# c0rv4x/zkevm-prover

Measured on AMD Instinct MI355X. Metric: batch-proof STARK sec (2^23 trace) + Goldilocks NTT Gelem/s at 1/2/4/8 GPU, lower is better.
Workload: dtype u64 (Goldilocks) + F_p^3

## Files before the change

### include/zkgpu.h

```cpp
#ifndef ZKGPU_H
#define ZKGPU_H

#include <stdint.h>
#include "zkgpu_zxp.h"

#ifdef __cplusplus
extern "C" {
#endif

#define ZKGPU_OK 0
#define ZKGPU_ERR_HIP -1
#define ZKGPU_ERR_ARG -2
#define ZKGPU_ERR_INIT -3
#define ZKGPU_ERR_OOM -4

int zkgpu_init(int device);
void zkgpu_release(void);
const char *zkgpu_last_error(void);
int zkgpu_set_stream(void *hip_stream);
void *zkgpu_get_stream(void);
int zkgpu_synchronize(void);
int zkgpu_abi_version(void);

int zkgpu_gl_ntt(uint64_t *dst, const uint64_t *src, uint64_t n, uint64_t ncols, int inverse);
// ... 126 lines not shown
                         const uint64_t *evals, uint32_t n_evals, char *buf, uint64_t buflen, int rtc_check);

int zkgpu_calculate_z_dev(uint64_t *z, uint64_t z_ld, const uint64_t *num, uint64_t num_ld, const uint64_t *den,
                          uint64_t den_ld, uint64_t n, int *closes);
int zkgpu_calculate_z_block_dev(uint64_t *z, uint64_t z_ld, const uint64_t *num, uint64_t num_ld, const uint64_t *den,
                                uint64_t den_ld, uint64_t n, const uint64_t z0[3], uint64_t total[3]);
typedef struct zkgpu_z_req {
    uint64_t *z;
    uint64_t z_ld;
    const uint64_t *num;
    uint64_t num_ld;
    const uint64_t *den;
    uint64_t den_ld;
} zkgpu_z_req;
int zkgpu_calculate_z_many_dev(const zkgpu_z_req *req, uint32_t nz, uint64_t n, int *closes);

int zkgpu_evmap_dev(uint64_t *evals_out, const uint64_t *const *cols, const uint64_t *lds, const uint32_t *dims,
                    const uint32_t *primes, uint32_t n_ev, const uint64_t *lev, const uint64_t *lpev, uint64_t l_ld,
                    uint64_t n, uint32_t extend_bits);

int zkgpu_xdivxsub_dev(uint64_t *xdiv, uint64_t *xdivw, const uint64_t xi[3], uint32_t n_bits, uint32_t n_bits_ext);
int zkgpu_xdivxsub_rows_dev(uint64_t *xdiv, uint64_t *xdivw, const uint64_t xi[3], uint32_t n_bits,
                            uint32_t n_bits_ext, uint64_t row0, uint64_t nrows);
int zkgpu_lagrange_xi_rows_dev(uint64_t *lev, uint64_t *lpev, uint64_t ld, const uint64_t xi[3], uint32_t n_bits,
                               uint64_t row0, uint64_t nrows);

int zkgpu_ext_powers_dev(uint64_t *out, uint64_t ld, const uint64_t base[3], uint64_t n);

int zkgpu_scale_by_powers_dev(uint64_t *cols, uint64_t ld, uint32_t ncols, uint64_t n, uint64_t base);

// ... 64 lines not shown
```

### zkevm-prover_amd/csrc/api.hip

```cpp
#include <stdarg.h>
#include <stdio.h>
#include <string.h>

#include <algorithm>
#include <deque>
#include <map>
#include <mutex>
#include <new>
#include <thread>
#include <vector>

#include "gl_device.hpp"
#include "zkgpu_internal.hpp"
#include "poseidon_gl_constants.h"
#include "poseidon_gl_sparse.h"

namespace zk {

int upload_poseidon_constants(Ctx &c);
int merkle_leaves_absorb(uint64_t *nodes, const uint64_t *src, uint64_t ld, uint64_t col0, uint64_t ncols,
                         uint64_t total, uint64_t nrows, hipStream_t s);

static Ctx g_ctx;
static thread_local char g_err[512] = "";
// ... 1164 lines not shown
int zkgpu_calculate_z_block_dev(uint64_t *z, uint64_t z_ld, const uint64_t *num, uint64_t num_ld, const uint64_t *den,
                                uint64_t den_ld, uint64_t n, const uint64_t z0[3], uint64_t total[3])
{
    int rc;
    if ((rc = require_init())) return rc;
    if (!z0 || !total) return set_error(ZKGPU_ERR_ARG, "calculate_z_block: null z0 / total");
    if (!n) {
        for (int k = 0; k < 3; k++) total[k] = z0[k] % HP;
        return 0;
    }
    if (z_ld < n || num_ld < n || den_ld < n) return set_error(ZKGPU_ERR_ARG, "calculate_z: ld < n");
    const size_t words = calculate_z_scratch_words(n);
    uint64_t *scr = workspace(2, (words + 8) * sizeof(uint64_t));
    if (!scr) return ZKGPU_ERR_OOM;
    uint64_t *tot = scr + words;
    if ((rc = calculate_z(z, z_ld, num, num_ld, den, den_ld, n, z0, scr, tot, g_ctx.stream))) return rc;
    if ((rc = check_hip(hipMemcpyAsync(total, tot, 24, hipMemcpyDeviceToHost, g_ctx.stream), "D2H"))) return rc;
    return check_hip(hipStreamSynchronize(g_ctx.stream), "calculateZ sync");
}

int zkgpu_calculate_z_many_dev(const zkgpu_z_req *req, uint32_t nz, uint64_t n, int *closes)
{
    int rc;
    if ((rc = require_init())) return rc;
    if (!nz) return 0;
    if (!req || !closes) return set_error(ZKGPU_ERR_ARG, "calculate_z_many: null argument");
    if (!n) {
        for (uint32_t k = 0; k < nz; k++) closes[k] = 1;
        return 0;
    }
    for (uint32_t k = 0; k < nz; k++)
        if (req[k].z_ld < n || req[k].num_ld < n || req[k].den_ld < n)
            return set_error(ZKGPU_ERR_ARG, "calculate_z_many: request %u: ld < n", k);
    const size_t words = calculate_z_scratch_words(n);
    uint64_t *scr = workspace(2, (words + 3ULL * nz + 8) * sizeof(uint64_t));
    if (!scr) return ZKGPU_ERR_OOM;
    uint64_t *tot = scr + words;
    const uint64_t one[3] = {1, 0, 0};
    for (uint32_t k = 0; k < nz; k++)
        if ((rc = calculate_z(req[k].z, req[k].z_ld, req[k].num, req[k].num_ld, req[k].den, req[k].den_ld, n, one, scr,
                              tot + 3ULL * k, g_ctx.stream)))
            return rc;
    std::vector<uint64_t> t(3ULL * nz);
    if ((rc = check_hip(hipMemcpyAsync(t.data(), tot, t.size() * 8, hipMemcpyDeviceToHost, g_ctx.stream), "D2H")))
        return rc;
    if ((rc = check_hip(hipStreamSynchronize(g_ctx.stream), "calculateZ sync"))) return rc;
    for (uint32_t k = 0; k < nz; k++) closes[k] = (t[3 * k] == 1 && t[3 * k + 1] == 0 && t[3 * k + 2] == 0) ? 1 : 0;
    return 0;
}

int zkgpu_calculate_z_dev(uint64_t *z, uint64_t z_ld, const uint64_t *num, uint64_t num_ld, const uint64_t *den,
                          uint64_t den_ld, uint64_t n, int *closes)
{
    const uint64_t one[3] = {1, 0, 0};
    uint64_t tot[3] = {1, 0, 0};
    const int rc = zkgpu_calculate_z_block_dev(z, z_ld, num, num_ld, den, den_ld, n, one, tot);
    if (rc) return rc;
// ... 490 lines not shown
```

### zkevm-prover_amd/csrc/stark.hip

```cpp
#include "gl_device.hpp"
#include "zkgpu_internal.hpp"
#include "../../include/zkgpu_zxp.h"

namespace zk {

template <int K>
__device__ __forceinline__ uint64_t sqr_n(uint64_t x)
{
#pragma unroll
    for (int i = 0; i < K; i++) x = gl_sqr(x);
    return x;
}

__device__ __forceinline__ uint64_t gl_inv_base(uint64_t x)
{
    uint64_t t2 = gl_mul(gl_sqr(x), x);
    uint64_t t3 = gl_mul(gl_sqr(t2), x);
    uint64_t t6 = gl_mul(sqr_n<3>(t3), t3);
    uint64_t t12 = gl_mul(sqr_n<6>(t6), t6);
    uint64_t t24 = gl_mul(sqr_n<12>(t12), t12);
    uint64_t t30 = gl_mul(sqr_n<6>(t24), t6);
    uint64_t t31 = gl_mul(gl_sqr(t30), x);
    uint64_t t32 = gl_mul(gl_sqr(t31), x);
    return gl_mul(sqr_n<33>(t31), t32);
}

__device__ __forceinline__ gl3 gl3_inv(const gl3 &a)
{
    uint64_t a0 = a.v[0], a1 = a.v[1], a2 = a.v[2];
    uint64_t s02 = gl_add(a0, a2), s12 = gl_add(a1, a2);
    uint64_t c0 = gl_sub(gl_mul(s02, s02), gl_mul(s12, a1));
    uint64_t c1 = gl_sub(gl_mul(s12, a2), gl_mul(a1, s02));
    uint64_t c2 = gl_sub(gl_mul(a1, a1), gl_mul(s02, a2));
    uint64_t det = gl_add(gl_add(gl_mul(a0, c0), gl_mul(a2, c1)), gl_mul(a1, c2));
    uint64_t di = gl_inv_base(det);
    return gl3{{gl_mul(c0, di), gl_mul(c1, di), gl_mul(c2, di)}};
}

__device__ __forceinline__ gl3 ld3(const uint64_t *p0, uint64_t ld)
{
    return gl3{{p0[0], p0[ld], p0[2 * ld]}};
}

__device__ __forceinline__ void st3(uint64_t *p0, uint64_t ld, const gl3 &v)
{
    p0[0] = gl_canon(v.v[0]);
    p0[ld] = gl_canon(v.v[1]);
    p0[2 * ld] = gl_canon(v.v[2]);
}

__device__ __forceinline__ uint64_t rand_u64(uint64_t seed, uint64_t stream, uint64_t col, uint64_t row)
// ... 282 lines not shown
__global__ void __launch_bounds__(ZXP_THREADS) k_zxp_eval_rows(ZxpEnv e, const uint64_t *rows, uint32_t n_rows)
{
    extern __shared__ __attribute__((aligned(16))) uint64_t zlds[];
    const int lane = threadIdx.x;
    const uint64_t j = (uint64_t)blockIdx.x * ZXP_THREADS + lane;
    const uint64_t i = j < n_rows ? rows[j] : ~0ULL;
    const bool active = i < (1ULL << e.logdom);
    if (!__ballot(active)) return;
    zxp_eval_body<true>(e, zlds, lane, i, active, j);
}

constexpr int BI_CHUNK = 16;
constexpr int SCAN_THREADS = 256;
constexpr int Z_PER = 4;
constexpr uint64_t Z_TILE = SCAN_THREADS * Z_PER;
__device__ __forceinline__ int z_slot(int e) { return e + e / Z_PER; }
constexpr int Z_SLOTS = Z_TILE + Z_TILE / Z_PER;

__device__ gl3 block_exclusive_scan3(gl3 v, gl3 *sh, gl3 *total)
{
    const int t = threadIdx.x;
    sh[t] = v;
    __syncthreads();
    for (int off = 1; off < SCAN_THREADS; off <<= 1) {
        gl3 x = sh[t];
        gl3 y = t >= off ? sh[t - off] : gl3{{1, 0, 0}};
        __syncthreads();
        sh[t] = t >= off ? gl3_mul(x, y) : x;
        __syncthreads();
    }
    gl3 excl = t ? sh[t - 1] : gl3{{1, 0, 0}};
    *total = sh[SCAN_THREADS - 1];
    __syncthreads();
    return excl;
}

__device__ __forceinline__ void lds_st3(uint64_t *img, int slot, const gl3 &v)
{
    img[slot] = v.v[0];
    img[Z_SLOTS + slot] = v.v[1];
    img[2 * Z_SLOTS + slot] = v.v[2];
}
__device__ __forceinline__ gl3 lds_ld3(const uint64_t *img, int slot)
{
    return gl3{{img[slot], img[Z_SLOTS + slot], img[2 * Z_SLOTS + slot]}};
}

__global__ void __launch_bounds__(SCAN_THREADS) k_z_ratio(uint64_t *ratio, uint64_t *thr_pre, uint64_t *tile_tot,
                                                          const uint64_t *num, uint64_t num_ld, const uint64_t *den,
                                                          uint64_t den_ld, uint64_t n)
{
    __shared__ uint64_t img[3 * Z_SLOTS];
    __shared__ gl3 sh[SCAN_THREADS];
    const int t = threadIdx.x;
    const uint64_t base = (uint64_t)blockIdx.x * Z_TILE;
    gl3 pre[Z_PER];
    gl3 acc{{1, 0, 0}};
#pragma unroll
    for (int j = 0; j < Z_PER; j++) {
        const uint64_t k = base + j * SCAN_THREADS + t;
        const gl3 d = k < n ? ld3(den + k, den_ld) : gl3{{1, 0, 0}};
        acc = j ? gl3_mul(acc, d) : d;
        pre[j] = acc;
    }
    gl3 inv = gl3_inv(acc);
#pragma unroll
    for (int jj = 0; jj < Z_PER; jj++) {
        const int j = Z_PER - 1 - jj;
        const int e = j * SCAN_THREADS + t;
        const uint64_t k = base + e;
        const gl3 dinv = j ? gl3_mul(inv, pre[j - 1]) : inv;
        gl3 r{{1, 0, 0}};
        if (k < n) {
            r = gl3_mul(ld3(num + k, num_ld), dinv);
            uint64_t *o = ratio + 3 * k;
            o[0] = r.v[0];
            o[1] = r.v[1];
            o[2] = r.v[2];
            if (j) inv = gl3_mul(inv, ld3(den + k, den_ld));
        }
        lds_st3(img, z_slot(e), r);
    }
    __syncthreads();
    gl3 run = lds_ld3(img, z_slot(t * Z_PER));
#pragma unroll
    for (int i = 1; i < Z_PER; i++) run = gl3_mul(run, lds_ld3(img, z_slot(t * Z_PER + i)));
    gl3 tot;
    const gl3 ex = block_exclusive_scan3(run, sh, &tot);
    uint64_t *tp = thr_pre + 3 * ((uint64_t)blockIdx.x * SCAN_THREADS + t);
    tp[0] = ex.v[0];
    tp[1] = ex.v[1];
    tp[2] = ex.v[2];
    if (t == 0) {
        tile_tot[3 * blockIdx.x] = tot.v[0];
        tile_tot[3 * blockIdx.x + 1] = tot.v[1];
        tile_tot[3 * blockIdx.x + 2] = tot.v[2];
    }
}

__global__ void __launch_bounds__(SCAN_THREADS) k_z_totals(uint64_t *tile_pre, const uint64_t *tile_tot,
                                                           uint64_t ntiles, gl3 z0, uint64_t *total)
{
    __shared__ gl3 sh[SCAN_THREADS];
    const uint64_t per = (ntiles + SCAN_THREADS - 1) / SCAN_THREADS;
    const uint64_t b0 = threadIdx.x * per;
    uint64_t b1 = b0 + per;
    if (b1 > ntiles) b1 = ntiles;
    gl3 acc{{1, 0, 0}};
    for (uint64_t b = b0; b < b1; b++) acc = gl3_mul(acc, ld3(tile_tot + 3 * b, 1));
    gl3 tot;
    gl3 run = gl3_mul(z0, block_exclusive_scan3(acc, sh, &tot));
    for (uint64_t b = b0; b < b1; b++) {
        tile_pre[3 * b] = run.v[0];
        tile_pre[3 * b + 1] = run.v[1];
        tile_pre[3 * b + 2] = run.v[2];
        run = gl3_mul(run, ld3(tile_tot + 3 * b, 1));
    }
    if (threadIdx.x == 0) {
        const gl3 t = gl3_canon(gl3_mul(z0, tot));
        total[0] = t.v[0];
        total[1] = t.v[1];
        total[2] = t.v[2];
    }
}

__global__ void __launch_bounds__(SCAN_THREADS) k_z_apply(uint64_t *z, uint64_t z_ld, const uint64_t *ratio,
                                                          const uint64_t *thr_pre, const uint64_t *tile_pre,
                                                          uint64_t n)
{
    __shared__ uint64_t img[3 * Z_SLOTS];
    const int t = threadIdx.x;
    const uint64_t base = (uint64_t)blockIdx.x * Z_TILE;
#pragma unroll
    for (int j = 0; j < Z_PER; j++) {
        const int e = j * SCAN_THREADS + t;
        const uint64_t k = base + e;
        lds_st3(img, z_slot(e), k < n ? ld3(ratio + 3 * k, 1) : gl3{{1, 0, 0}});
    }
    gl3 run = gl3_mul(ld3(tile_pre + 3 * blockIdx.x, 1), ld3(thr_pre + 3 * ((uint64_t)blockIdx.x * SCAN_THREADS + t), 1));
    __syncthreads();
#pragma unroll
    for (int i = 0; i < Z_PER; i++) {
        const int sl = z_slot(t * Z_PER + i);
        const gl3 r = lds_ld3(img, sl);
        lds_st3(img, sl, run);
        run = gl3_mul(run, r);
    }
    __syncthreads();
#pragma unroll
    for (int j = 0; j < Z_PER; j++) {
        const int e = j * SCAN_THREADS + t;
        const uint64_t k = base + e;
        if (k < n) st3(z + k, z_ld, lds_ld3(img, z_slot(e)));
    }
}

constexpr int EV_THREADS = 256;

constexpr int EV_G = 8;
constexpr uint64_t EV_ROWS_PER_THREAD = 240;
struct EvGroup {
    const uint64_t *col[EV_G];
    uint32_t prime, sub0;
};

template <int G, int U>
__global__ void __launch_bounds__(EV_THREADS) k_evmap_groups(uint64_t *partial, const EvGroup *groups,
                                                            const uint64_t *lev, const uint64_t *lpev, uint64_t l_ld,
// ... 66 lines not shown
    }
    acc = gl3_canon(acc);
    evals[3 * e] = acc.v[0];
    evals[3 * e + 1] = acc.v[1];
    evals[3 * e + 2] = acc.v[2];
}

template <bool INTERLEAVED>
__global__ void __launch_bounds__(256) k_xdiv_rows(uint64_t *out0, uint64_t *out1, uint64_t ld, gl3 a0, gl3 a1,
                                                   uint64_t shift, gl3 scale, uint32_t logn, uint64_t row0,
                                                   uint64_t nrows, const uint64_t *tw_lo, const uint64_t *tw_hi)
{
    const uint64_t n = 1ULL << logn;
    const uint64_t T = (uint64_t)gridDim.x * blockDim.x;
    const uint64_t t = (uint64_t)blockIdx.x * blockDim.x + threadIdx.x;
    for (int which = 0; which < 2; which++) {
        const gl3 s = which ? a1 : a0;
        uint64_t *out = which ? out1 : out0;
        gl3 pre[BI_CHUNK];
        uint64_t xs[BI_CHUNK];
        gl3 acc{{1, 0, 0}};
#pragma unroll
        for (int j = 0; j < BI_CHUNK; j++) {
            uint64_t k = t + j * T;
            uint64_t ex = ((row0 + k) & (n - 1)) << (TW_MAX_LOG - logn);
            xs[j] = gl_mul(shift, gl_mul(tw_lo[ex & (TW_LEVEL_SIZE - 1)], tw_hi[ex >> TW_LEVEL_BITS]));
            gl3 d = k < nrows ? gl3{{gl_sub(xs[j], s.v[0]), gl_neg(s.v[1]), gl_neg(s.v[2])}} : gl3{{1, 0, 0}};
            acc = j ? gl3_mul(acc, d) : d;
            pre[j] = acc;
        }
        gl3 inv = gl3_inv(acc);
#pragma unroll
        for (int jj = 0; jj < BI_CHUNK; jj++) {
            const int j = BI_CHUNK - 1 - jj;
            uint64_t k = t + j * T;
            gl3 dinv = j ? gl3_mul(inv, pre[j - 1]) : inv;
            if (k < nrows) {
                gl3 d{{gl_sub(xs[j], s.v[0]), gl_neg(s.v[1]), gl_neg(s.v[2])}};
                gl3 r = gl3_mul1(dinv, xs[j]);
                if constexpr (!INTERLEAVED) r = gl3_mul(r, scale);
                r = gl3_canon(r);
                if constexpr (INTERLEAVED) {
                    out[3 * k] = r.v[0];
                    out[3 * k + 1] = r.v[1];
                    out[3 * k + 2] = r.v[2];
                } else {
                    out[k] = r.v[0];
                    out[ld + k] = r.v[1];
                    out[2 * ld + k] = r.v[2];
                }
                inv = gl3_mul(inv, d);
            }
        }
    }
}

__device__ __forceinline__ gl3 gl3_pow(gl3 b, uint64_t e)
{
    gl3 r{{1, 0, 0}};
    while (e) {
        if (e & 1) r = gl3_mul(r, b);
        b = gl3_mul(b, b);
        e >>= 1;
    }
    return r;
}
// ... 132 lines not shown
    if (!n_rows) return 0;
    size_t lds;
    const ZxpEnv e = zxp_env(L, true, lds);
    prof_begin(s);
    hipLaunchKernelGGL(k_zxp_eval_rows, dim3(nblk(n_rows, ZXP_THREADS)), dim3(ZXP_THREADS), lds, s, e, rows, n_rows);
    prof_end("k_zxp_eval_rows", L.bytes, s);
    return check_launch("k_zxp_eval_rows");
}

size_t calculate_z_scratch_words(uint64_t n)
{
    const uint64_t nt = (n + Z_TILE - 1) / Z_TILE;
    return 3 * n + 3 * nt * SCAN_THREADS + 6 * nt + 4;
}

int calculate_z(uint64_t *z, uint64_t z_ld, const uint64_t *num, uint64_t num_ld, const uint64_t *den,
                uint64_t den_ld, uint64_t n, const uint64_t z0[3], uint64_t *scratch, uint64_t *total_dev, hipStream_t s)
{
    const uint64_t nt = (n + Z_TILE - 1) / Z_TILE;
    uint64_t *ratio = scratch;
    uint64_t *thr = ratio + 3 * n;
    uint64_t *tot = thr + 3 * nt * SCAN_THREADS;
    uint64_t *pre = tot + 3 * nt;
    prof_begin(s);
    hipLaunchKernelGGL(k_z_ratio, dim3((uint32_t)nt), dim3(SCAN_THREADS), 0, s, ratio, thr, tot, num, num_ld, den,
                       den_ld, n);
    prof_end("k_z_ratio", 8.0 * 9 * n, s);
    const gl3 z0v{{z0[0], z0[1], z0[2]}};
    hipLaunchKernelGGL(k_z_totals, dim3(1), dim3(SCAN_THREADS), 0, s, pre, tot, nt, z0v, total_dev);
    prof_begin(s);
    hipLaunchKernelGGL(k_z_apply, dim3((uint32_t)nt), dim3(SCAN_THREADS), 0, s, z, z_ld, ratio, thr, pre, n);
    prof_end("k_z_apply", 8.0 * 6 * n, s);
    return check_launch("calculateZ");
}

size_t evmap_group_size() { return sizeof(EvGroup); }
uint32_t evmap_group_width() { return EV_G; }
uint64_t evmap_rows_per_block() { return EV_ROWS_PER_THREAD * EV_THREADS; }

int evmap_groups(uint64_t *evals, const void *groups_dev, uint32_t n_groups, uint32_t width, uint32_t unroll,
                 const int32_t *subs_dev,
                 uint32_t n_ev, uint32_t n_sub, const uint64_t *lev, const uint64_t *lpev, uint64_t l_ld, uint64_t n,
                 uint32_t eb, uint64_t *partial, hipStream_t s)
{
    if (!n_ev) return 0;
    const uint64_t rpb = evmap_rows_per_block();
    const uint32_t nblk_ = (uint32_t)((n + rpb - 1) / rpb);
// ... 117 lines not shown
```

### zkevm-prover_amd/csrc/zkgpu_internal.hpp

```cpp
#pragma once
#include <hip/hip_runtime.h>
#include <stdint.h>

#include "../../include/zkgpu.h"
#include "../../include/zkgpu_zxp.h"
#include "zxp_jit_source.hpp"
#include "zxp_prepare.hpp"

namespace zk {

constexpr uint32_t NTT_MAX_PASSES = 4;
constexpr uint32_t POST_BITS = 12;

struct Workspace {
    void *ptr = nullptr;
    size_t bytes = 0;
};

struct Ctx {
    int device = -1;
    bool ready = false;
    hipStream_t stream = nullptr;
    uint64_t *rt_small[2] = {nullptr, nullptr};
    uint64_t *tw_lo[2] = {nullptr, nullptr};
// ... 50 lines not shown
int fri_fold_rows(uint64_t *out, const uint64_t *rows, uint64_t g0, uint64_t n_local, uint32_t pol_bits,
                  uint32_t out_bits, const uint64_t sx[3], uint64_t shift_inv, hipStream_t s);
int fri_transpose(uint64_t *aux, const uint64_t *pol, uint64_t degree, uint32_t tbits, hipStream_t s);

int zxp_jit_run(const ZxpJitIn &in, hipStream_t s);

int rand_cols(uint64_t *base, uint64_t ld, const uint32_t *cols_dev, uint32_t ncols, uint64_t nrows, uint64_t seed,
              uint64_t stream, uint64_t row0, uint64_t rmask, hipStream_t s);
int copy_rows(uint64_t *dst, uint64_t dld, uint64_t drow0, const uint32_t *dcols, const uint64_t *src, uint64_t sld,
              uint64_t srow0, uint64_t smask, const uint32_t *scols, uint32_t ncols, uint64_t nrows, hipStream_t s);
int zxp_eval(const ZxpLaunch &L, hipStream_t s);
int zxp_eval_rows(const ZxpLaunch &L, const uint64_t *rows, uint32_t n_rows, hipStream_t s);
uint32_t nonzero_rows_blocks(uint64_t n);
int nonzero_rows(uint64_t *out, uint32_t *counts, const uint64_t *cols, uint64_t ld, uint32_t ncols, uint64_t n,
                 uint32_t max_rows, hipStream_t s);
size_t calculate_z_scratch_words(uint64_t n);
int calculate_z(uint64_t *z, uint64_t z_ld, const uint64_t *num, uint64_t num_ld, const uint64_t *den,
                uint64_t den_ld, uint64_t n, const uint64_t z0[3], uint64_t *scratch, uint64_t *total_dev, hipStream_t s);
size_t evmap_group_size();
uint32_t evmap_group_width();
uint64_t evmap_rows_per_block();
int evmap_groups(uint64_t *evals, const void *groups_dev, uint32_t n_groups, uint32_t width, uint32_t unroll,
                 const int32_t *subs_dev,
                 uint32_t n_ev, uint32_t n_sub, const uint64_t *lev, const uint64_t *lpev, uint64_t l_ld, uint64_t n, uint32_t eb,
                 uint64_t *partial, hipStream_t s);
int xdivxsub(uint64_t *xdiv, uint64_t *xdivw, const uint64_t xi[3], uint64_t w, uint32_t logn, hipStream_t s);
int xdivxsub_rows(uint64_t *xdiv, uint64_t *xdivw, const uint64_t xi[3], uint64_t w, uint32_t logn, uint64_t row0,
                  uint64_t nrows, hipStream_t s);
int xdiv_rows(uint64_t *out0, uint64_t *out1, uint64_t ld, int interleaved, const uint64_t a0[3],
              const uint64_t a1[3], uint64_t shift, const uint64_t scale[3], uint32_t logn, uint64_t row0,
              uint64_t nrows, hipStream_t s);
int ext_powers(uint64_t *out, uint64_t ld, const uint64_t base[3], uint64_t n, hipStream_t s);
int scale_powers(uint64_t *cols, uint64_t ld, uint32_t ncols, uint64_t n, uint64_t base, hipStream_t s);
// ... 14 lines not shown
```

### zkevm-prover_amd/host/sharded_starks.hpp

```cpp

class ShardedStarks : public Starks
{
public:
    zkgpu_comm comm{};
    uint32_t W = 1, R = 0;
    uint64_t B = 0, H = 0, BH = 0;
    uint64_t hn = 0, ldn = 0;
    uint64_t *ext = nullptr;
    uint64_t *coln = nullptr;
    uint64_t *gath = nullptr;
    uint64_t *cm4 = nullptr;
    uint64_t *xchg = nullptr;
    uint64_t *hsend = nullptr, *hrecv = nullptr;
    uint64_t *pack_s = nullptr, *pack_r = nullptr;
    uint64_t *psend(uint32_t d) const { return pack_s + (uint64_t)(d < R ? d : d - 1) * stride_s; }
    uint64_t stride_s = 0, stride_r = 0;
    uint32_t max_ops = 0;
    uint64_t n_exch = 0, sent_bytes = 0, max_sent = 0;
    uint64_t *puw = nullptr;
    uint64_t *hs_send = nullptr, *hs_recv = nullptr, *hs_ret = nullptr, *hs_ret_in = nullptr, *hs_seg = nullptr;
    uint32_t *hs_cnt = nullptr, *hs_start = nullptr;
    uint64_t hs_recv_cap = 0;
    uint64_t slot = 0, hcap = 0;
    struct Tree {
// ... 181 lines not shown
        return 8 * ((coln_words() >= const_words() ? 0 : const_words()) + (ext_words() >= const_words() ? 0 : const_words()));
    }
    int setup_buffer(uint64_t **p, uint64_t *have, uint64_t cap, uint64_t words, void **owned)
    {
        *owned = nullptr;
        if (have && cap >= words) {
            *p = have;
            return 0;
        }
        CK(zkgpu_dev_malloc(owned, words * 8));
        *p = (uint64_t *)*owned;
        return 0;
    }
    uint64_t lde_cols_max() const override { return max_share(); }
    uint64_t prog_rows_max() const override { return std::max(B, nb); }

    uint64_t s0_record() const
    {
        return (uint64_t)info.n_cm1 + info.n_cm2 + info.n_cm3 + info.n_cm4 + info.n_const + 20ULL * info.n_bits_ext;
    }

    int exchange()
    {
        if (W == 1) {
            ops.clear();
            return 0;
        }
        max_ops = std::max(max_ops, (uint32_t)ops.size());
        if (ops.size() > 2ULL * (W - 1)) {
            const size_t n = ops.size();
// ... 850 lines not shown
```

### zkevm-prover_amd/host/starks.cpp

```cpp
#include <math.h>
#include <stdarg.h>
#include <stdio.h>
#include <stdlib.h>
#include <string.h>

#include <algorithm>
#include <chrono>
#include <map>
#include <string>
#include <vector>

#include "../../include/zkgpu.h"
#include "../../include/zkgpu_stark.h"
#include "zkgpu_audit_format.hpp"

namespace zkgpu_host {

static thread_local char g_err[512] = "";
static int fail(const char *fmt, ...)
{
    va_list ap;
    va_start(ap, fmt);
    vsnprintf(g_err, sizeof g_err, fmt, ap);
    va_end(ap);
// ... 179 lines not shown
        }
        void *v = nullptr;
        CK(zkgpu_dev_malloc(&v, elems * 8));
        allocs.push_back(v);
        CK(zkgpu_memset_dev(v, 0, elems * 8));
        *p = (uint64_t *)v;
        return 0;
    }

    virtual uint64_t setup_bytes() const { return 0; }
    virtual uint64_t lde_cols_max() const
    {
        return std::max({info.n_cm1, info.n_cm2, info.n_cm3, info.n_const, 1u});
    }
    virtual uint64_t prog_rows_max() const { return NE; }
    virtual uint64_t stream_stage_words() const
    {
        const uint64_t b = std::min<uint64_t>(std::max(info.n_cm1, 1u), 128);
        return 2 * std::min<uint64_t>(N * b, (64ULL << 20) / 8);
    }
    uint64_t lde_batch_cap = 0;
    int plan(uint64_t *bytes)
    {
        dry = true;
        planned = 0;
        const int rc = alloc();
        dry = false;
        if (rc) return -1;
        const uint64_t ntt_ws = std::max<uint64_t>(3, info.n_cm4) * NE * 8;
        const uint64_t lde_ws = zkgpu_lde_workspace_bytes(
            N, NE, lde_batch_cap ? std::min<uint64_t>(lde_cols_max(), lde_batch_cap) : lde_cols_max());
        const uint64_t prog_ws = 64ULL * prog_rows_max() * 8;
        const uint64_t h1h2_ws = info.n_pu ? 32ULL * N : 0;
        *bytes = planned + setup_bytes() + std::max(lde_ws, ntt_ws + zkgpu_lde_workspace_bytes(N, NE, 0)) + prog_ws +
                 h1h2_ws + 24ULL * N +
                 stream_stage_words() * 8;
        planned = 0;
        return 0;
    }
    int check_budget()
    {
        uint64_t need = 0, avail = 0, total = 0;
        if (plan(&need)) return -1;
        CK(zkgpu_device_memory(&avail, &total));
        if (need > avail)
            return fail("stark_create: this prover needs %.1f GB of HBM per GPU (%u-row trace, %u/%u/%u/%u committed "
                        "columns, %u constants), the device has %.1f GB free of %.1f GB",
                        need / 1e9, (unsigned)N, info.n_cm1, info.n_cm2, info.n_cm3, info.n_cm4, info.n_const,
                        avail / 1e9, total / 1e9);
        return 0;
    }
// ... 1193 lines not shown
                                (unsigned long long)miss, k);
                return fail("calculateH1H2: %s", zkgpu_last_error());
            }
        }
        return 0;
    }

    std::vector<zkgpu_z_req> z_requests() const
    {
        std::vector<zkgpu_z_req> req(info.n_zctx);
        for (uint32_t z = 0; z < info.n_zctx; z++)
            req[z] = {S.sec[SEC_CM3_N] + (uint64_t)zctx[3 * z + 2] * N, N, S.sec[SEC_TMP_N] + (uint64_t)zctx[3 * z] * N, N,
                      S.sec[SEC_TMP_N] + (uint64_t)zctx[3 * z + 1] * N, N};
        return req;
    }
    virtual int z_all()
    {
        const std::vector<zkgpu_z_req> req = z_requests();
        std::vector<int> closes(info.n_zctx + 1, 0);
        CK(zkgpu_calculate_z_many_dev(req.data(), info.n_zctx, N, closes.data()));
        uint32_t n_open = 0, first = 0;
        for (uint32_t z = info.n_zctx; z-- > 0;)
            if (!closes[z]) n_open++, first = z;
        return n_open ? z_open(first, n_open) : 0;
    }

    zkgpu_z_diag zdiag = {};

    int z_open(uint32_t z, uint32_t n_open)
    {
        zdiag = zkgpu_z_diag{};
        zdiag.z = z;
        zdiag.n_open = n_open;
        std::string why;
        if (!z_compare(z, zdiag.n_num, zdiag.n_den, zdiag.num, zdiag.den, why))
// ... 228 lines not shown
                if (!rc) continue;
                if (miss == ~0ULL) return fail("audit: calculateH1H2: %s", zkgpu_last_error());
                CK(zkgpu_memset_dev(h1, 0, (uint64_t)q[4] * N * 8));
                CK(zkgpu_memset_dev(h2, 0, (uint64_t)q[4] * N * 8));
                if (R.n_pu_bad++ < ZKGPU_AUDIT_MAX_PU && audit_misses(k, R.pu[R.n_pu_bad - 1])) return -1;
            }
            if (tstop("AUDIT_H1H2")) return -1;
        }
        tstart();
        if (run(step3prev, false, ch, ev0, 0)) return -1;
        if (tstop("AUDIT_STEP3PREV")) return -1;
        tstart();
        {
            const std::vector<zkgpu_z_req> req = z_requests();
            std::vector<int> closes(info.n_zctx + 1, 0);
            CK(zkgpu_calculate_z_many_dev(req.data(), info.n_zctx, N, closes.data()));
            for (uint32_t z = 0; z < info.n_zctx; z++) {
                if (closes[z]) continue;
                if (R.n_z_open++ >= ZKGPU_AUDIT_MAX_Z) continue;
                zkgpu_audit_z &e = R.z[R.n_z_open - 1];
                e.z = z;
                std::string why;
                e.compared = z_compare(z, e.n_num, e.n_den, e.num, e.den, why);
                const auto it = conns.find(z);
                if (it != conns.end()) (void)conn_run(z, it->second, audit_conns[R.n_z_open - 1], why);
            }
        }
        if (tstop("AUDIT_Z")) return -1;
        if (R.n_z_open) {
            const zkgpu_audit_z &e = R.z[0];
            zdiag.ran = e.compared;
// ... 487 lines not shown
```

### zkevm-prover_amd/zkgpu/__init__.py

```python
import ctypes
import os
import subprocess

import numpy as np

_HERE = os.path.dirname(os.path.abspath(__file__))
PKG_ROOT = os.path.dirname(_HERE)
LIB_DIR = os.environ.get("ZKGPU_LIB_DIR") or os.path.join(PKG_ROOT, "lib")
LIB_PATH = os.path.join(LIB_DIR, "libzkgpu.so")
HEADER = os.path.join(os.path.dirname(PKG_ROOT), "include", "zkgpu.h")

P = 0xFFFFFFFF00000001


class ZkgpuError(RuntimeError):
    pass


_lib = None

u64 = ctypes.c_uint64
u32 = ctypes.c_uint32
vp = ctypes.c_void_p
pu64 = ctypes.POINTER(ctypes.c_uint64)
# ... 81 lines not shown
    "zkgpu_multiset_diff_workspace_bytes": (u64, [u64]),
    "zkgpu_multiset_diff_dev": (ctypes.c_int, [vp, vp, u64, vp, u64, u64, u32, u32]),
    "zkgpu_lookup_misses_workspace_bytes": (u64, [u64]),
    "zkgpu_lookup_misses_dev": (ctypes.c_int, [vp, vp, u64, vp, u64, u64, u32, u32]),
    "zkgpu_conn_breaks_workspace_bytes": (u64, [u64, u32]),
    "zkgpu_conn_ks_check": (ctypes.c_int, [vp, u32, u32]),
    "zkgpu_conn_breaks_dev": (ctypes.c_int, [vp, vp, u64, vp, vp, u64, vp, u32, vp, u32, u32]),
    "zkgpu_h1h2_shard_route": (ctypes.c_int, [vp, u64, vp, vp, vp, u64, vp, u64, u64, u64, u32, u32]),
    "zkgpu_h1h2_shard_owner": (ctypes.c_int, [vp, vp, u64, u32, pu64]),
    "zkgpu_h1h2_shard_counts": (ctypes.c_int, [vp, vp, pu64, vp, vp, u64, u64, u64]),
    "zkgpu_h1h2_shard_deal": (ctypes.c_int, [vp, u64, vp, u64, vp, vp, u64, u32]),
    "zkgpu_h1h2_shard_place": (ctypes.c_int, [vp, u64, vp, u64, vp, u64, u64, u64, u64, u32]),
    "zkgpu_gl_merkle_open_rows_dev": (ctypes.c_int, [vp, vp, vp, vp, u64, u64, vp, u64]),
    "zkgpu_gl_merkle_open_many": (ctypes.c_int, [vp, u32]),
    "zkgpu_calculate_z_many_dev": (ctypes.c_int, [vp, u32, u64, vp]),
    "zkgpu_prof_enable": (ctypes.c_int, [ctypes.c_int]),
    "zkgpu_prof_reset": (ctypes.c_int, []),
    "zkgpu_prof_query": (ctypes.c_int, [ctypes.c_char_p, pu64, ctypes.POINTER(ctypes.c_double),
                                        ctypes.POINTER(ctypes.c_double)]),
    "zkgpu_prof_kernels": (ctypes.c_int, [ctypes.c_char_p, u64]),
    "zkgpu_mark": (ctypes.c_int, [u32]),
    "zkgpu_mark_elapsed": (ctypes.c_int, [u32, u32, ctypes.POINTER(ctypes.c_double)]),
    "zkgpu_exec_create": (ctypes.c_int, [ctypes.POINTER(vp), vp, u64, u64, u32]),
    "zkgpu_exec_info": (ctypes.c_int, [vp, pu64, pu64, ctypes.POINTER(u32), ctypes.POINTER(u32), pu64]),
    "zkgpu_exec_commit_dev": (ctypes.c_int, [vp, vp, vp, u64, u64]),
    "zkgpu_exec_destroy": (None, [vp]),
    "zkgpu_exec_set_tail_width": (None, [u32]),
    "zkgpu_parser_convert": (ctypes.c_int, [u32, vp, u64, vp, u64, vp, u32, u32, u32, vp]),
    "zkgpu_steps_parser_eval": (ctypes.c_int, [u32, vp, u64, vp, u64, vp, u32, u32, u32, vp]),
    "zkgpu_steps_mirror": (ctypes.c_int, [ctypes.c_int]),
# ... 824 lines not shown
```

Measured before the change: 0.2220.

## Batch grand-product Z computations and invert via base-field determinants

Grand-product Z computation now runs several products per launch through a 2D grid with per-product scratch, replacing one three-kernel sequence per product. The F_p^3 batch inversion now inverts only base-field determinants (adjugate times inverse determinant), sharing one Montgomery-style inversion across four values per wave. Block scans use wave shuffles instead of LDS ping-pong. The xdiv kernel gets the same determinant-based inversion with hoisted twiddle computation. Together these cut launch count and field-inverse cost, at the price of a larger workspace (capped at 2 GiB) and more complex kernels.

```diff
diff --git a/include/zkgpu.h b/include/zkgpu.h
--- a/include/zkgpu.h
+++ b/include/zkgpu.h
@@ -164,6 +164,7 @@
     uint64_t den_ld;
 } zkgpu_z_req;
 int zkgpu_calculate_z_many_dev(const zkgpu_z_req *req, uint32_t nz, uint64_t n, int *closes);
+uint64_t zkgpu_calculate_z_workspace_bytes(uint64_t n, uint32_t nz);
 
 int zkgpu_evmap_dev(uint64_t *evals_out, const uint64_t *const *cols, const uint64_t *lds, const uint32_t *dims,
                     const uint32_t *primes, uint32_t n_ev, const uint64_t *lev, const uint64_t *lpev, uint64_t l_ld,
diff --git a/zkevm-prover_amd/csrc/api.hip b/zkevm-prover_amd/csrc/api.hip
--- a/zkevm-prover_amd/csrc/api.hip
+++ b/zkevm-prover_amd/csrc/api.hip
@@ -1202,9 +1202,23 @@
     uint64_t *scr = workspace(2, (words + 8) * sizeof(uint64_t));
     if (!scr) return ZKGPU_ERR_OOM;
     uint64_t *tot = scr + words;
-    if ((rc = calculate_z(z, z_ld, num, num_ld, den, den_ld, n, z0, scr, tot, g_ctx.stream))) return rc;
+    const ZProduct one_product{z, z_ld, num, num_ld, den, den_ld, {z0[0], z0[1], z0[2]}, tot};
+    if ((rc = calculate_z(&one_product, 1, n, scr, g_ctx.stream))) return rc;
     if ((rc = check_hip(hipMemcpyAsync(total, tot, 24, hipMemcpyDeviceToHost, g_ctx.stream), "D2H"))) return rc;
     return check_hip(hipStreamSynchronize(g_ctx.stream), "calculateZ sync");
+}
+
+constexpr uint64_t Z_BATCH_BYTES = 2ULL << 30;
+static uint32_t z_batch(uint64_t n, uint32_t nz)
+{
+    const uint64_t fit = Z_BATCH_BYTES / (calculate_z_scratch_words(n) * sizeof(uint64_t));
+    return (uint32_t)std::max<uint64_t>(1, std::min<uint64_t>({(uint64_t)nz, (uint64_t)Z_MAX_BATCH, fit}));
+}
+
+uint64_t zkgpu_calculate_z_workspace_bytes(uint64_t n, uint32_t nz)
+{
+    if (!n || !nz) return 0;
+    return (calculate_z_scratch_words(n) * z_batch(n, nz) + 3ULL * nz + 8) * sizeof(uint64_t);
 }
 
 int zkgpu_calculate_z_many_dev(const zkgpu_z_req *req, uint32_t nz, uint64_t n, int *closes)
@@ -1221,14 +1235,19 @@
         if (req[k].z_ld < n || req[k].num_ld < n || req[k].den_ld < n)
             return set_error(ZKGPU_ERR_ARG, "calculate_z_many: request %u: ld < n", k);
     const size_t words = calculate_z_scratch_words(n);
-    uint64_t *scr = workspace(2, (words + 3ULL * nz + 8) * sizeof(uint64_t));
+    const uint32_t batch = z_batch(n, nz);
+    uint64_t *scr = workspace(2, (words * batch + 3ULL * nz + 8) * sizeof(uint64_t));
     if (!scr) return ZKGPU_ERR_OOM;
-    uint64_t *tot = scr + words;
-    const uint64_t one[3] = {1, 0, 0};
-    for (uint32_t k = 0; k < nz; k++)
-        if ((rc = calculate_z(req[k].z, req[k].z_ld, req[k].num, req[k].num_ld, req[k].den, req[k].den_ld, n, one, scr,
-                              tot + 3ULL * k, g_ctx.stream)))
-            return rc;
+    uint64_t *tot = scr + words * batch;
+    for (uint32_t k0 = 0; k0 < nz; k0 += batch) {
+        ZProduct p[Z_MAX_BATCH];
+        const uint32_t nb = std::min(batch, nz - k0);
+        for (uint32_t i = 0; i < nb; i++) {
+            const zkgpu_z_req &r = req[k0 + i];
+            p[i] = ZProduct{r.z, r.z_ld, r.num, r.num_ld, r.den, r.den_ld, {1, 0, 0}, tot + 3ULL * (k0 + i)};
+        }
+        if ((rc = calculate_z(p, nb, n, scr, g_ctx.stream))) return rc;
+    }
     std::vector<uint64_t> t(3ULL * nz);
     if ((rc = check_hip(hipMemcpyAsync(t.data(), tot, t.size() * 8, hipMemcpyDeviceToHost, g_ctx.stream), "D2H")))
         return rc;
diff --git a/zkevm-prover_amd/csrc/stark.hip b/zkevm-prover_amd/csrc/stark.hip
--- a/zkevm-prover_amd/csrc/stark.hip
+++ b/zkevm-prover_amd/csrc/stark.hip
@@ -25,16 +25,15 @@
     return gl_mul(sqr_n<33>(t31), t32);
 }
 
-__device__ __forceinline__ gl3 gl3_inv(const gl3 &a)
+__device__ __forceinline__ gl3 gl3_adj_det(const gl3 &a, uint64_t *det)
 {
     uint64_t a0 = a.v[0], a1 = a.v[1], a2 = a.v[2];
     uint64_t s02 = gl_add(a0, a2), s12 = gl_add(a1, a2);
     uint64_t c0 = gl_sub(gl_mul(s02, s02), gl_mul(s12, a1));
     uint64_t c1 = gl_sub(gl_mul(s12, a2), gl_mul(a1, s02));
     uint64_t c2 = gl_sub(gl_mul(a1, a1), gl_mul(s02, a2));
-    uint64_t det = gl_add(gl_add(gl_mul(a0, c0), gl_mul(a2, c1)), gl_mul(a1, c2));
-    uint64_t di = gl_inv_base(det);
-    return gl3{{gl_mul(c0, di), gl_mul(c1, di), gl_mul(c2, di)}};
+    *det = gl_add(gl_add(gl_mul(a0, c0), gl_mul(a2, c1)), gl_mul(a1, c2));
+    return gl3{{c0, c1, c2}};
 }
 
 __device__ __forceinline__ gl3 ld3(const uint64_t *p0, uint64_t ld)
@@ -347,25 +346,69 @@
 constexpr int SCAN_THREADS = 256;
 constexpr int Z_PER = 4;
 constexpr uint64_t Z_TILE = SCAN_THREADS * Z_PER;
+constexpr int Z_WAVES = SCAN_THREADS / 64;
+static_assert(Z_WAVES == 4 && Z_PER == 4, "k_z_ratio's one-wave steps take 4 products / 4 runs per lane");
 __device__ __forceinline__ int z_slot(int e) { return e + e / Z_PER; }
 constexpr int Z_SLOTS = Z_TILE + Z_TILE / Z_PER;
 
-__device__ gl3 block_exclusive_scan3(gl3 v, gl3 *sh, gl3 *total)
-{
-    const int t = threadIdx.x;
-    sh[t] = v;
-    __syncthreads();
-    for (int off = 1; off < SCAN_THREADS; off <<= 1) {
-        gl3 x = sh[t];
-        gl3 y = t >= off ? sh[t - off] : gl3{{1, 0, 0}};
-        __syncthreads();
-        sh[t] = t >= off ? gl3_mul(x, y) : x;
-        __syncthreads();
-    }
-    gl3 excl = t ? sh[t - 1] : gl3{{1, 0, 0}};
-    *total = sh[SCAN_THREADS - 1];
-    __syncthreads();
-    return excl;
+struct ZReq {
+    uint64_t *z;
+    const uint64_t *num, *den;
+    uint64_t z_ld, num_ld, den_ld;
+    gl3 z0;
+    uint64_t *total;
+};
+struct ZBatch {
+    ZReq r[Z_MAX_BATCH];
+    uint64_t *scratch;
+    uint64_t words;
+};
+struct ZScratch {
+    uint64_t *ratio, *thr, *tot, *pre;
+};
+__device__ __forceinline__ ZScratch z_scratch(const ZBatch &b, uint64_t n, uint64_t nt)
+{
+    ZScratch s;
+    s.ratio = b.scratch + blockIdx.y * b.words;
+    s.thr = s.ratio + 3 * n;
+    s.tot = s.thr + 3 * nt * SCAN_THREADS;
+    s.pre = s.tot + 3 * nt;
+    return s;
+}
+
+__device__ __forceinline__ gl3 shfl_up3(const gl3 &v, int off)
+{
+    return gl3{{__shfl_up(v.v[0], off), __shfl_up(v.v[1], off), __shfl_up(v.v[2], off)}};
+}
+
+__device__ __forceinline__ gl3 wave_inclusive_scan3(gl3 v)
+{
+    const int lane = threadIdx.x & 63;
+#pragma unroll
+    for (int off = 1; off < 64; off <<= 1) {
+        const gl3 m = gl3_mul(shfl_up3(v, off), v);
+        if (lane >= off) v = m;
+    }
+    return v;
+}
+
+__device__ gl3 block_exclusive_scan3(gl3 v, gl3 *wt, gl3 *total)
+{
+    const int lane = threadIdx.x & 63, w = threadIdx.x >> 6;
+    const gl3 inc = wave_inclusive_scan3(v);
+    if (lane == 63) wt[w] = inc;
+    gl3 ex = shfl_up3(inc, 1);
+    if (lane == 0) ex = gl3{{1, 0, 0}};
+    __syncthreads();
+    gl3 run{{1, 0, 0}};
+#pragma unroll
+    for (int i = 0; i < Z_WAVES; i++) {
+        if (i == w) ex = gl3_mul(run, ex);
+        run = gl3_mul(run, wt[i]);
+    }
+    *total = run;
+    __syncthreads();
+    return ex;
 }
 
 __device__ __forceinline__ void lds_st3(uint64_t *img, int slot, const gl3 &v)
@@ -379,98 +422,143 @@
     return gl3{{img[slot], img[Z_SLOTS + slot], img[2 * Z_SLOTS + slot]}};
 }
 
-__global__ void __launch_bounds__(SCAN_THREADS) k_z_ratio(uint64_t *ratio, uint64_t *thr_pre, uint64_t *tile_tot,
-                                                          const uint64_t *num, uint64_t num_ld, const uint64_t *den,
-                                                          uint64_t den_ld, uint64_t n)
+__device__ __forceinline__ int z_worker(int step)
+{
+    const uint32_t i = blockIdx.x >> 3;
+    return (int)((i + (i >> 2) + (i >> 5) + (i >> 7) + blockIdx.y + step) & (Z_WAVES - 1));
+}
+
+__global__ void __launch_bounds__(SCAN_THREADS) k_z_ratio(const ZBatch b, uint64_t n, uint64_t nt)
 {
     __shared__ uint64_t img[3 * Z_SLOTS];
     __shared__ gl3 sh[SCAN_THREADS];
-    const int t = threadIdx.x;
+    uint64_t *shp = (uint64_t *)sh;
+    const ZReq q = b.r[blockIdx.y];
+    const ZScratch scr = z_scratch(b, n, nt);
+    const int t = threadIdx.x, lane = t & 63, w = t >> 6;
     const uint64_t base = (uint64_t)blockIdx.x * Z_TILE;
-    gl3 pre[Z_PER];
-    gl3 acc{{1, 0, 0}};
+    gl3 c[Z_PER], nm[Z_PER];
+    uint64_t e[Z_PER], pre[Z_PER];
+    uint64_t acc = 1;
+    bool zero = false;
 #pragma unroll
     for (int j = 0; j < Z_PER; j++) {
         const uint64_t k = base + j * SCAN_THREADS + t;
-        const gl3 d = k < n ? ld3(den + k, den_ld) : gl3{{1, 0, 0}};
-        acc = j ? gl3_mul(acc, d) : d;
+        const gl3 d = k < n ? ld3(q.den + k, q.den_ld) : gl3{{1, 0, 0}};
+        nm[j] = k < n ? ld3(q.num + k, q.num_ld) : gl3{{1, 0, 0}};
+        uint64_t det;
+        c[j] = gl3_adj_det(d, &det);
+        const bool z = gl_canon(det) == 0;
+        zero |= z;
+        e[j] = z ? 1 : det;
+        acc = j ? gl_mul(acc, e[j]) : e[j];
         pre[j] = acc;
     }
-    gl3 inv = gl3_inv(acc);
+    shp[t] = acc;
+    __syncthreads();
+    if (w == z_worker(0)) {
+        const uint64_t q0 = shp[lane], q1 = shp[64 + lane], q2 = shp[128 + lane], q3 = shp[192 + lane];
+        const uint64_t p01 = gl_mul(q0, q1), p012 = gl_mul(p01, q2);
+        uint64_t inv = gl_inv_base(gl_mul(p012, q3));
+        shp[192 + lane] = gl_mul(inv, p012);
+        inv = gl_mul(inv, q3);
+        shp[128 + lane] = gl_mul(inv, p01);
+        inv = gl_mul(inv, q2);
+        shp[64 + lane] = gl_mul(inv, q0);
+        shp[lane] = gl_mul(inv, q1);
+    }
+    __syncthreads();
+    uint64_t inv = zero ? 0 : shp[t];
 #pragma unroll
     for (int jj = 0; jj < Z_PER; jj++) {
         const int j = Z_PER - 1 - jj;
-        const int e = j * SCAN_THREADS + t;
-        const uint64_t k = base + e;
-        const gl3 dinv = j ? gl3_mul(inv, pre[j - 1]) : inv;
+        const int el = j * SCAN_THREADS + t;
+        const uint64_t k = base + el;
+        const uint64_t di = j ? gl_mul(inv, pre[j - 1]) : inv;
         gl3 r{{1, 0, 0}};
         if (k < n) {
-            r = gl3_mul(ld3(num + k, num_ld), dinv);
-            uint64_t *o = ratio + 3 * k;
+            r = gl3_mul(nm[j], gl3_mul1(c[j], di));
+            uint64_t *o = scr.ratio + 3 * k;
             o[0] = r.v[0];
             o[1] = r.v[1];
             o[2] = r.v[2];
-            if (j) inv = gl3_mul(inv, ld3(den + k, den_ld));
-        }
-        lds_st3(img, z_slot(e), r);
+        }
+        if (j) inv = gl_mul(inv, e[j]);
+        lds_st3(img, z_slot(el), r);
     }
     __syncthreads();
     gl3 run = lds_ld3(img, z_slot(t * Z_PER));
 #pragma unroll
     for (int i = 1; i < Z_PER; i++) run = gl3_mul(run, lds_ld3(img, z_slot(t * Z_PER + i)));
-    gl3 tot;
-    const gl3 ex = block_exclusive_scan3(run, sh, &tot);
-    uint64_t *tp = thr_pre + 3 * ((uint64_t)blockIdx.x * SCAN_THREADS + t);
+    sh[t] = run;
+    __syncthreads();
+    if (w == z_worker(2)) {
+        const gl3 r0 = sh[4 * lane], r1 = sh[4 * lane + 1], r2 = sh[4 * lane + 2], r3 = sh[4 * lane + 3];
+        const gl3 p1 = gl3_mul(r0, r1), p2 = gl3_mul(p1, r2);
+        const gl3 inc = wave_inclusive_scan3(gl3_mul(p2, r3));
+        gl3 ex = shfl_up3(inc, 1);
+        if (lane == 0) ex = gl3{{1, 0, 0}};
+        sh[4 * lane] = ex;
+        sh[4 * lane + 1] = gl3_mul(ex, r0);
+        sh[4 * lane + 2] = gl3_mul(ex, p1);
+        sh[4 * lane + 3] = gl3_mul(ex, p2);
+        if (lane == 63) {
+            scr.tot[3 * blockIdx.x] = inc.v[0];
+            scr.tot[3 * blockIdx.x + 1] = inc.v[1];
+            scr.tot[3 * blockIdx.x + 2] = inc.v[2];
+        }
+    }
+    __syncthreads();
+    const gl3 ex = sh[t];
+    uint64_t *tp = scr.thr + 3 * ((uint64_t)blockIdx.x * SCAN_THREADS + t);
     tp[0] = ex.v[0];
     tp[1] = ex.v[1];
     tp[2] = ex.v[2];
-    if (t == 0) {
-        tile_tot[3 * blockIdx.x] = tot.v[0];
-        tile_tot[3 * blockIdx.x + 1] = tot.v[1];
-        tile_tot[3 * blockIdx.x + 2] = tot.v[2];
-    }
-}
-
-__global__ void __launch_bounds__(SCAN_THREADS) k_z_totals(uint64_t *tile_pre, const uint64_t *tile_tot,
-                                                           uint64_t ntiles, gl3 z0, uint64_t *total)
-{
-    __shared__ gl3 sh[SCAN_THREADS];
+}
+
+__global__ void __launch_bounds__(SCAN_THREADS) k_z_totals(const ZBatch b, uint64_t n, uint64_t ntiles)
+{
+    __shared__ gl3 wt[Z_WAVES];
+    const ZReq q = b.r[blockIdx.y];
+    const ZScratch scr = z_scratch(b, n, ntiles);
+    const uint64_t *tile_tot = scr.tot;
+    uint64_t *tile_pre = scr.pre;
     const uint64_t per = (ntiles + SCAN_THREADS - 1) / SCAN_THREADS;
     const uint64_t b0 = threadIdx.x * per;
     uint64_t b1 = b0 + per;
     if (b1 > ntiles) b1 = ntiles;
     gl3 acc{{1, 0, 0}};
-    for (uint64_t b = b0; b < b1; b++) acc = gl3_mul(acc, ld3(tile_tot + 3 * b, 1));
+    for (uint64_t i = b0; i < b1; i++) acc = gl3_mul(acc, ld3(tile_tot + 3 * i, 1));
     gl3 tot;
-    gl3 run = gl3_mul(z0, block_exclusive_scan3(acc, sh, &tot));
-    for (uint64_t b = b0; b < b1; b++) {
-        tile_pre[3 * b] = run.v[0];
-        tile_pre[3 * b + 1] = run.v[1];
-        tile_pre[3 * b + 2] = run.v[2];
-        run = gl3_mul(run, ld3(tile_tot + 3 * b, 1));
+    gl3 run = gl3_mul(q.z0, block_exclusive_scan3(acc, wt, &tot));
+    for (uint64_t i = b0; i < b1; i++) {
+        tile_pre[3 * i] = run.v[0];
+        tile_pre[3 * i + 1] = run.v[1];
+        tile_pre[3 * i + 2] = run.v[2];
+        run = gl3_mul(run, ld3(tile_tot + 3 * i, 1));
     }
     if (threadIdx.x == 0) {
-        const gl3 t = gl3_canon(gl3_mul(z0, tot));
-        total[0] = t.v[0];
-        total[1] = t.v[1];
-        total[2] = t.v[2];
-    }
-}
-
-__global__ void __launch_bounds__(SCAN_THREADS) k_z_apply(uint64_t *z, uint64_t z_ld, const uint64_t *ratio,
-                                                          const uint64_t *thr_pre, const uint64_t *tile_pre,
-                                                          uint64_t n)
+        const gl3 t = gl3_canon(gl3_mul(q.z0, tot));
+        q.total[0] = t.v[0];
+        q.total[1] = t.v[1];
+        q.total[2] = t.v[2];
+    }
+}
+
+__global__ void __launch_bounds__(SCAN_THREADS) k_z_apply(const ZBatch b, uint64_t n, uint64_t nt)
 {
     __shared__ uint64_t img[3 * Z_SLOTS];
+    const ZReq q = b.r[blockIdx.y];
+    const ZScratch scr = z_scratch(b, n, nt);
     const int t = threadIdx.x;
     const uint64_t base = (uint64_t)blockIdx.x * Z_TILE;
 #pragma unroll
     for (int j = 0; j < Z_PER; j++) {
         const int e = j * SCAN_THREADS + t;
         const uint64_t k = base + e;
-        lds_st3(img, z_slot(e), k < n ? ld3(ratio + 3 * k, 1) : gl3{{1, 0, 0}});
-    }
-    gl3 run = gl3_mul(ld3(tile_pre + 3 * blockIdx.x, 1), ld3(thr_pre + 3 * ((uint64_t)blockIdx.x * SCAN_THREADS + t), 1));
+        lds_st3(img, z_slot(e), k < n ? ld3(scr.ratio + 3 * k, 1) : gl3{{1, 0, 0}});
+    }
+    gl3 run = gl3_mul(ld3(scr.pre + 3 * blockIdx.x, 1), ld3(scr.thr + 3 * ((uint64_t)blockIdx.x * SCAN_THREADS + t), 1));
     __syncthreads();
 #pragma unroll
     for (int i = 0; i < Z_PER; i++) {
@@ -484,7 +572,7 @@
     for (int j = 0; j < Z_PER; j++) {
         const int e = j * SCAN_THREADS + t;
         const uint64_t k = base + e;
-        if (k < n) st3(z + k, z_ld, lds_ld3(img, z_slot(e)));
+        if (k < n) st3(q.z + k, q.z_ld, lds_ld3(img, z_slot(e)));
     }
 }
 
@@ -581,32 +669,47 @@
     const uint64_t n = 1ULL << logn;
     const uint64_t T = (uint64_t)gridDim.x * blockDim.x;
     const uint64_t t = (uint64_t)blockIdx.x * blockDim.x + threadIdx.x;
+    uint64_t xs[BI_CHUNK];
+#pragma unroll
+    for (int j = 0; j < BI_CHUNK; j++) {
+        const uint64_t ex = ((row0 + t + j * T) & (n - 1)) << (TW_MAX_LOG - logn);
+        xs[j] = gl_mul(shift, gl_mul(tw_lo[ex & (TW_LEVEL_SIZE - 1)], tw_hi[ex >> TW_LEVEL_BITS]));
+    }
+#pragma unroll 1
     for (int which = 0; which < 2; which++) {
         const gl3 s = which ? a1 : a0;
         uint64_t *out = which ? out1 : out0;
-        gl3 pre[BI_CHUNK];
-        uint64_t xs[BI_CHUNK];
-        gl3 acc{{1, 0, 0}};
+        const uint64_t d1 = gl_neg(s.v[1]), d2 = gl_neg(s.v[2]), s12 = gl_add(d1, d2);
+        const uint64_t k0 = gl_mul(s12, d1), k1 = gl_mul(s12, d2), k2 = gl_mul(d1, d1);
+        const uint64_t k3 = gl_add(gl_mul(d2, k1), gl_mul(d1, k2)), k4 = gl_mul(gl_add(d1, d1), d2);
+        const uint64_t ub = gl_sub(d2, s.v[0]);
+        uint64_t pre[BI_CHUNK], dets[BI_CHUNK];
+        uint64_t acc = 1;
 #pragma unroll
         for (int j = 0; j < BI_CHUNK; j++) {
-            uint64_t k = t + j * T;
-            uint64_t ex = ((row0 + k) & (n - 1)) << (TW_MAX_LOG - logn);
-            xs[j] = gl_mul(shift, gl_mul(tw_lo[ex & (TW_LEVEL_SIZE - 1)], tw_hi[ex >> TW_LEVEL_BITS]));
-            gl3 d = k < nrows ? gl3{{gl_sub(xs[j], s.v[0]), gl_neg(s.v[1]), gl_neg(s.v[2])}} : gl3{{1, 0, 0}};
-            acc = j ? gl3_mul(acc, d) : d;
+            const uint64_t k = t + j * T;
+            const uint64_t u = gl_add(xs[j], ub);
+            const uint64_t c0 = gl_sub(gl_mul(u, u), k0);
+            const uint64_t det = gl_sub(gl_add(gl_mul(gl_sub(u, d2), c0), k3), gl_mul(k4, u));
+            dets[j] = k < nrows ? det : 1;
+            acc = j ? gl_mul(acc, dets[j]) : dets[j];
             pre[j] = acc;
         }
-        gl3 inv = gl3_inv(acc);
+        uint64_t inv = gl_inv_base(acc);
 #pragma unroll
         for (int jj = 0; jj < BI_CHUNK; jj++) {
             const int j = BI_CHUNK - 1 - jj;
-            uint64_t k = t + j * T;
-            gl3 dinv = j ? gl3_mul(inv, pre[j - 1]) : inv;
+            const uint64_t k = t + j * T;
+            uint64_t x = xs[j];
+            asm volatile("" : "+v"(x), "+v"(inv));
+            const uint64_t dinv = j ? gl_mul(inv, pre[j - 1]) : inv;
+            inv = gl_mul(inv, dets[j]);
+            const uint64_t u = gl_add(x, ub);
+            const gl3 c{{gl_sub(gl_mul(u, u), k0), gl_sub(k1, gl_mul(d1, u)), gl_sub(k2, gl_mul(d2, u))}};
+            gl3 r = gl3_mul1(c, gl_mul(dinv, x));
+            if constexpr (!INTERLEAVED) r = gl3_mul(r, scale);
+            r = gl3_canon(r);
             if (k < nrows) {
-                gl3 d{{gl_sub(xs[j], s.v[0]), gl_neg(s.v[1]), gl_neg(s.v[2])}};
-                gl3 r = gl3_mul1(dinv, xs[j]);
-                if constexpr (!INTERLEAVED) r = gl3_mul(r, scale);
-                r = gl3_canon(r);
                 if constexpr (INTERLEAVED) {
                     out[3 * k] = r.v[0];
                     out[3 * k + 1] = r.v[1];
@@ -616,7 +719,6 @@
                     out[ld + k] = r.v[1];
                     out[2 * ld + k] = r.v[2];
                 }
-                inv = gl3_mul(inv, d);
             }
         }
     }
@@ -779,23 +881,26 @@
     return 3 * n + 3 * nt * SCAN_THREADS + 6 * nt + 4;
 }
 
-int calculate_z(uint64_t *z, uint64_t z_ld, const uint64_t *num, uint64_t num_ld, const uint64_t *den,
-                uint64_t den_ld, uint64_t n, const uint64_t z0[3], uint64_t *scratch, uint64_t *total_dev, hipStream_t s)
-{
+int calculate_z(const ZProduct *p, uint32_t nz, uint64_t n, uint64_t *scratch, hipStream_t s)
+{
+    if (!nz || nz > Z_MAX_BATCH) return set_error(ZKGPU_ERR_ARG, "calculate_z: %u products in one batch", nz);
     const uint64_t nt = (n + Z_TILE - 1) / Z_TILE;
-    uint64_t *ratio = scratch;
-    uint64_t *thr = ratio + 3 * n;
-    uint64_t *tot = thr + 3 * nt * SCAN_THREADS;
-    uint64_t *pre = tot + 3 * nt;
+    ZBatch b{};
+    for (uint32_t k = 0; k < nz; k++)
+        b.r[k] = ZReq{p[k].z, p[k].num, p[k].den, p[k].z_ld, p[k].num_ld, p[k].den_ld,
+                      gl3{{p[k].z0[0], p[k].z0[1], p[k].z0[2]}}, p[k].total_dev};
+    b.scratch = scratch;
+    b.words = calculate_z_scratch_words(n);
+    const dim3 tiles((uint32_t)nt, nz);
     prof_begin(s);
-    hipLaunchKernelGGL(k_z_ratio, dim3((uint32_t)nt), dim3(SCAN_THREADS), 0, s, ratio, thr, tot, num, num_ld, den,
-                       den_ld, n);
-    prof_end("k_z_ratio", 8.0 * 9 * n, s);
-    const gl3 z0v{{z0[0], z0[1], z0[2]}};
-    hipLaunchKernelGGL(k_z_totals, dim3(1), dim3(SCAN_THREADS), 0, s, pre, tot, nt, z0v, total_dev);
+    hipLaunchKernelGGL(k_z_ratio, tiles, dim3(SCAN_THREADS), 0, s, b, n, nt);
+    prof_end("k_z_ratio", 8.0 * 9 * n * nz, s);
     prof_begin(s);
-    hipLaunchKernelGGL(k_z_apply, dim3((uint32_t)nt), dim3(SCAN_THREADS), 0, s, z, z_ld, ratio, thr, pre, n);
-    prof_end("k_z_apply", 8.0 * 6 * n, s);
+    hipLaunchKernelGGL(k_z_totals, dim3(1, nz), dim3(SCAN_THREADS), 0, s, b, n, nt);
+    prof_end("k_z_totals", 8.0 * 6 * nt * nz, s);
+    prof_begin(s);
+    hipLaunchKernelGGL(k_z_apply, tiles, dim3(SCAN_THREADS), 0, s, b, n, nt);
+    prof_end("k_z_apply", 8.0 * 6 * n * nz, s);
     return check_launch("calculateZ");
 }
 
diff --git a/zkevm-prover_amd/csrc/zkgpu_internal.hpp b/zkevm-prover_amd/csrc/zkgpu_internal.hpp
--- a/zkevm-prover_amd/csrc/zkgpu_internal.hpp
+++ b/zkevm-prover_amd/csrc/zkgpu_internal.hpp
@@ -88,9 +88,19 @@
 uint32_t nonzero_rows_blocks(uint64_t n);
 int nonzero_rows(uint64_t *out, uint32_t *counts, const uint64_t *cols, uint64_t ld, uint32_t ncols, uint64_t n,
                  uint32_t max_rows, hipStream_t s);
+constexpr uint32_t Z_MAX_BATCH = 16;
+struct ZProduct {
+    uint64_t *z;
+    uint64_t z_ld;
+    const uint64_t *num;
+    uint64_t num_ld;
+    const uint64_t *den;
+    uint64_t den_ld;
+    uint64_t z0[3];
+    uint64_t *total_dev;
+};
 size_t calculate_z_scratch_words(uint64_t n);
-int calculate_z(uint64_t *z, uint64_t z_ld, const uint64_t *num, uint64_t num_ld, const uint64_t *den,
-                uint64_t den_ld, uint64_t n, const uint64_t z0[3], uint64_t *scratch, uint64_t *total_dev, hipStream_t s);
+int calculate_z(const ZProduct *p, uint32_t nz, uint64_t n, uint64_t *scratch, hipStream_t s);
 size_t evmap_group_size();
 uint32_t evmap_group_width();
 uint64_t evmap_rows_per_block();
diff --git a/zkevm-prover_amd/host/sharded_starks.hpp b/zkevm-prover_amd/host/sharded_starks.hpp
--- a/zkevm-prover_amd/host/sharded_starks.hpp
+++ b/zkevm-prover_amd/host/sharded_starks.hpp
@@ -219,6 +219,7 @@
     }
     uint64_t lde_cols_max() const override { return max_share(); }
     uint64_t prog_rows_max() const override { return std::max(B, nb); }
+    uint64_t z_ws_bytes() const override { return 24ULL * N; }
 
     uint64_t s0_record() const
     {
diff --git a/zkevm-prover_amd/host/starks.cpp b/zkevm-prover_amd/host/starks.cpp
--- a/zkevm-prover_amd/host/starks.cpp
+++ b/zkevm-prover_amd/host/starks.cpp
@@ -217,6 +217,10 @@
         return std::max({info.n_cm1, info.n_cm2, info.n_cm3, info.n_const, 1u});
     }
     virtual uint64_t prog_rows_max() const { return NE; }
+    virtual uint64_t z_ws_bytes() const
+    {
+        return lean() ? 24ULL * N : std::max<uint64_t>(24ULL * N, zkgpu_calculate_z_workspace_bytes(N, info.n_zctx));
+    }
     virtual uint64_t stream_stage_words() const
     {
         const uint64_t b = std::min<uint64_t>(std::max(info.n_cm1, 1u), 128);
@@ -236,8 +240,7 @@
         const uint64_t prog_ws = 64ULL * prog_rows_max() * 8;
         const uint64_t h1h2_ws = info.n_pu ? 32ULL * N : 0;
         *bytes = planned + setup_bytes() + std::max(lde_ws, ntt_ws + zkgpu_lde_workspace_bytes(N, NE, 0)) + prog_ws +
-                 h1h2_ws + 24ULL * N +
-                 stream_stage_words() * 8;
+                 h1h2_ws + z_ws_bytes() + stream_stage_words() * 8;
         planned = 0;
         return 0;
     }
@@ -1461,11 +1464,17 @@
                       S.sec[SEC_TMP_N] + (uint64_t)zctx[3 * z + 1] * N, N};
         return req;
     }
+    int z_many(const std::vector<zkgpu_z_req> &req, std::vector<int> &closes)
+    {
+        if (!lean()) return zkgpu_calculate_z_many_dev(req.data(), info.n_zctx, N, closes.data());
+        for (uint32_t z = 0; z < info.n_zctx; z++) CK(zkgpu_calculate_z_many_dev(&req[z], 1, N, &closes[z]));
+        return 0;
+    }
     virtual int z_all()
     {
         const std::vector<zkgpu_z_req> req = z_requests();
         std::vector<int> closes(info.n_zctx + 1, 0);
-        CK(zkgpu_calculate_z_many_dev(req.data(), info.n_zctx, N, closes.data()));
+        CK(z_many(req, closes));
         uint32_t n_open = 0, first = 0;
         for (uint32_t z = info.n_zctx; z-- > 0;)
             if (!closes[z]) n_open++, first = z;
@@ -1724,7 +1733,7 @@
         {
             const std::vector<zkgpu_z_req> req = z_requests();
             std::vector<int> closes(info.n_zctx + 1, 0);
-            CK(zkgpu_calculate_z_many_dev(req.data(), info.n_zctx, N, closes.data()));
+            CK(z_many(req, closes));
             for (uint32_t z = 0; z < info.n_zctx; z++) {
                 if (closes[z]) continue;
                 if (R.n_z_open++ >= ZKGPU_AUDIT_MAX_Z) continue;
diff --git a/zkevm-prover_amd/zkgpu/__init__.py b/zkevm-prover_amd/zkgpu/__init__.py
--- a/zkevm-prover_amd/zkgpu/__init__.py
+++ b/zkevm-prover_amd/zkgpu/__init__.py
@@ -119,6 +119,7 @@
     "zkgpu_gl_merkle_open_rows_dev": (ctypes.c_int, [vp, vp, vp, vp, u64, u64, vp, u64]),
     "zkgpu_gl_merkle_open_many": (ctypes.c_int, [vp, u32]),
     "zkgpu_calculate_z_many_dev": (ctypes.c_int, [vp, u32, u64, vp]),
+    "zkgpu_calculate_z_workspace_bytes": (u64, [u64, u32]),
     "zkgpu_prof_enable": (ctypes.c_int, [ctypes.c_int]),
     "zkgpu_prof_reset": (ctypes.c_int, []),
     "zkgpu_prof_query": (ctypes.c_int, [ctypes.c_char_p, pu64, ctypes.POINTER(ctypes.c_double),
```

New measurement: 0.2203, median of 6. Within noise of the previous version (-0.8%).
